# LiqunZhao/Neural-ordinary-differential-equations-based-Lyapunov-Barrier-Actor-Critic-NLBAC

Measured on AMD Instinct MI355X. Metric: ODE-integrate+update samples/sec, Unicycle batch 4096, higher is better.
Workload: dtype f32; 1 GPU; Unicycle B=4096 dopri5 (BASELINE.json configs[1] at B=4096 dopri5); NODE fit on 32768 rows every 10 updates; replay of 65536 synthetic transitions resident in HBM; solver=dopri5, adjoint=False, batch_per_gpu=4096, global_batch=4096, node_fit_rows_per_gpu=32768, parallelism=dp1, hipgraph=False

## Files before the change

### neural-ordinary-differential-equations-based-lyapunov-barrier-actor-critic-nlbac_amd/csrc/mlp_kernels.hip

```cpp
#include "common.h"
#include "mlp_device.h"
#include "rr_device.h"
#include "dy_heads.h"
#include "mlp_launch.h"


__global__ __launch_bounds__(256) void mlp_pack_kernel(const MlpLaunch L) {
    const nlbac_mlp& net = L.net[blockIdx.y];
    const int nwide = net.n_layers - 1;
    const int hid = net.hid;
    const long gid = (long)blockIdx.x * 256 + threadIdx.x;
    const long stride = (long)gridDim.x * 256;
    for (int l = 0; l < nwide; ++l) {
        const int K = (l == 0) ? net.in_dim : hid;
        const float* W = net.params + net.w_off[l];
        if (net.pf_off[l] >= 0) {
            const int KC = pad8(K) >> 3, NT = pad32(hid) >> 5;
            float* P = net.packed + net.pf_off[l];
            const long total = (long)NT * KC * 256;
            for (long i = gid; i < total; i += stride) {
                const int j = i & 3, lane = (i >> 2) & 63;
                const long tc = i >> 8;
                const int kc = tc % KC, tile = tc / KC;
                const int n = 32 * tile + (lane & 31), k = 8 * kc + 4 * (lane >> 5) + j;
// ... 396 lines not shown
    for (int r = 0; r < 16; ++r) acc[r] = 0.f;

#define DW_LOAD(r0_, A0, A1, B0, B1)                                                        \
    {                                                                                       \
        const int ra_ = min((r0_) + lr, re - 1), rb_ = min((r0_) + lr + 16, re - 1);        \
        A0 = *reinterpret_cast<const float4*>(pa + (long)ra_ * hid);                        \
        A1 = *reinterpret_cast<const float4*>(pa + (long)rb_ * hid);                        \
        B0 = *reinterpret_cast<const float4*>(pb + (long)ra_ * hid);                        \
        B1 = *reinterpret_cast<const float4*>(pb + (long)rb_ * hid);                        \
    }
#define DW_STAGE(r0_, A0, A1, B0, B1, buf_)                                                 \
    {                                                                                       \
        const bool lo_ = (r0_) + lr < re, hi_ = (r0_) + lr + 16 < re;                       \
        *reinterpret_cast<float4*>(&sA[buf_][lr][lc]) = sel4(a_ok && lo_, A0);              \
        *reinterpret_cast<float4*>(&sA[buf_][lr + 16][lc]) = sel4(a_ok && hi_, A1);         \
        *reinterpret_cast<float4*>(&sB[buf_][lr][lc]) = sel4(b_ok && lo_, B0);              \
        *reinterpret_cast<float4*>(&sB[buf_][lr + 16][lc]) = sel4(b_ok && hi_, B1);         \
    }
#define DW_MFMA(buf_)                                                                       \
    {                                                                                       \
        float av[DW_CHUNK / 2], bv[DW_CHUNK / 2];                                           \
        _Pragma("unroll") for (int bb = 0; bb < DW_CHUNK / 2; ++bb) {                       \
            av[bb] = sA[buf_][2 * bb + half][wn * 32 + (lane & 31)];                        \
            bv[bb] = sB[buf_][2 * bb + half][wk * 32 + (lane & 31)];                        \
        }                                                                                   \
        __builtin_amdgcn_sched_barrier(0);                                                  \
        _Pragma("unroll") for (int bb = 0; bb < DW_CHUNK / 2; ++bb)                         \
            acc = __builtin_amdgcn_mfma_f32_32x32x2f32(av[bb], bv[bb], acc, 0, 0, 0);       \
    }
    if (rb < re) {
        float4 x_a0, x_a1, x_b0, x_b1, y_a0, y_a1, y_b0, y_b1;
        DW_LOAD(rb, x_a0, x_a1, x_b0, x_b1)
        DW_STAGE(rb, x_a0, x_a1, x_b0, x_b1, 0)
        DW_LOAD(rb + DW_CHUNK, x_a0, x_a1, x_b0, x_b1)
        __syncthreads();
        for (int r0 = rb; r0 < re; r0 += 2 * DW_CHUNK) {
            if (r0 + 2 * DW_CHUNK < re) DW_LOAD(r0 + 2 * DW_CHUNK, y_a0, y_a1, y_b0, y_b1)
            __builtin_amdgcn_sched_barrier(0);
            DW_MFMA(0)
            __builtin_amdgcn_sched_barrier(0);
            if (r0 + DW_CHUNK < re) DW_STAGE(r0 + DW_CHUNK, x_a0, x_a1, x_b0, x_b1, 1)
            __syncthreads();
            if (r0 + DW_CHUNK >= re) break;
            if (r0 + 3 * DW_CHUNK < re) DW_LOAD(r0 + 3 * DW_CHUNK, x_a0, x_a1, x_b0, x_b1)
            __builtin_amdgcn_sched_barrier(0);
            DW_MFMA(1)
            __builtin_amdgcn_sched_barrier(0);
            if (r0 + 2 * DW_CHUNK < re) DW_STAGE(r0 + 2 * DW_CHUNK, y_a0, y_a1, y_b0, y_b1, 0)
            __syncthreads();
        }
    }
    float* g = io.grad + (long)slab * L.slab_stride + net.w_off[j];
    const int k = k0 + wk * 32 + (lane & 31);
#pragma unroll
    for (int r = 0; r < 16; ++r) {
        const int n = n0 + wn * 32 + acc_row(r, half);
        if (n < hid && k < hid) g[(long)n * hid + k] = acc[r];
    }
}

#define DWT_PF 8
__global__ __launch_bounds__(256, 3) void mlp_bwd_wide64_kernel(const MlpLaunch L, const SkinnyLaunch S,
                                                                const float* __restrict__ ws, int red_blocks,
                                                                int red_per_net, int n_nets, int tiles_per_group) {
    extern __shared__ __attribute__((aligned(16))) float dwt_smem[];
    if ((int)blockIdx.x < red_blocks) {
        const int inet = blockIdx.x / red_per_net;
        if (inet < n_nets)
            skinny_reduce_block(L, S, ws, blockIdx.x - inet * red_per_net, inet, reinterpret_cast<float (*)[64]>(dwt_smem));
        return;
    }
    const int id = (int)blockIdx.x - red_blocks, xcd = id & 7, jj = id >> 3;
    const int t = jj % tiles_per_group, grp = 8 * (jj / tiles_per_group) + xcd;
    if (grp >= L.n_slabs * n_nets) return;
    const int znet = grp / L.n_slabs, slab = grp - znet * L.n_slabs;
    const nlbac_mlp& net = L.net[znet];
    const nlbac_mlp_io& io = L.io[znet];
    const int B = L.B, hid = net.hid, nwide = net.n_layers - 1;
    const int T = (hid + 63) >> 6, per_layer = T * T;
    if (t >= (nwide - 1) * per_layer) return;
    const int j = 1 + t / per_layer, tt = t % per_layer;
    const int n0 = (tt / T) * 64, k0 = (tt % T) * 64;
    const int rb = slab * L.rows_per_slab, re = min(B, rb + L.rows_per_slab);
    const int tid = threadIdx.x, lane = tid & 63, wave = tid >> 6, q = lane >> 4, i = lane & 15;
    const long ls = io.acts_ls ? io.acts_ls : (long)B * hid;
    const __amdgpu_buffer_rsrc_t rsA = rr_rsrc(io.dz + (long)j * ls, max(re, 0) * hid);
    const __amdgpu_buffer_rsrc_t rsB = rr_rsrc(io.acts + (long)(j - 1) * ls, max(re, 0) * hid);
    const int oob = (int)0x80000000;
    const int voA = (n0 + 4 * i + 3 < hid) ? (q * hid + n0 + 4 * i) * 4 : oob;
    const int voB = (k0 + 4 * i + 3 < hid) ? (q * hid + k0 + 4 * i) * 4 : oob;
    const int kstep_bytes = 16 * hid;
    const int g_first = (rb >> 2) + wave, n_mine = (rb < re) ? (((re - rb + 3) >> 2) - wave + 3) / 4 : 0;
    f32x4 acc[4][4];
#pragma unroll
    for (int ta = 0; ta < 4; ++ta)
#pragma unroll
        for (int tb = 0; tb < 4; ++tb) acc[ta][tb] = f32x4{0.f, 0.f, 0.f, 0.f};
    f32x4 va[DWT_PF], vb[DWT_PF];
    const int rounds = (n_mine + DWT_PF - 1) / DWT_PF;
    if (rounds > 0) {
#pragma unroll
        for (int u = 0; u < DWT_PF; ++u) {
            const int so = (g_first + 4 * u) * kstep_bytes;
            va[u] = rr_ldw(rsA, voA, so);
            vb[u] = rr_ldw(rsB, voB, so);
        }
        int g = g_first + 4 * DWT_PF;
        for (int r = 0; r < rounds; ++r) {
#pragma unroll
            for (int u = 0; u < DWT_PF; ++u) {
                const f32x4 a = va[u], b = vb[u];
#pragma unroll
                for (int ta = 0; ta < 4; ++ta)
#pragma unroll
                    for (int tb = 0; tb < 4; ++tb)
                        acc[ta][tb] = __builtin_amdgcn_mfma_f32_16x16x4f32(a[ta], b[tb], acc[ta][tb], 0, 0, 0);
                const int so = g * kstep_bytes;
                va[u] = rr_ldw(rsA, voA, so);
                vb[u] = rr_ldw(rsB, voB, so);
                __builtin_amdgcn_sched_barrier(0);
                g += 4;
            }
        }
    }
    float* const red0 = dwt_smem, * const red1 = dwt_smem + 64 * 64;
    auto put = [&](float* red) __attribute__((always_inline)) {
#pragma unroll
        for (int ta = 0; ta < 4; ++ta)
#pragma unroll
            for (int tb = 0; tb < 4; ++tb)
                *reinterpret_cast<f32x4*>(red + ((ta * 4 + tb) * 64 + lane) * 4) = acc[ta][tb];
    };
    auto add = [&](const float* red) __attribute__((always_inline)) {
#pragma unroll
        for (int ta = 0; ta < 4; ++ta)
#pragma unroll
            for (int tb = 0; tb < 4; ++tb) acc[ta][tb] += *reinterpret_cast<const f32x4*>(red + ((ta * 4 + tb) * 64 + lane) * 4);
    };
    if (wave == 1) put(red0);
    if (wave == 3) put(red1);
    lds_barrier();
    if (wave == 0) add(red0);
    if (wave == 2) add(red1);
    lds_barrier();
    if (wave == 2) put(red0);
    lds_barrier();
    if (wave != 0) return;
    add(red0);
    float* gW = io.grad + (long)slab * L.slab_stride + net.w_off[j];
    if (k0 + 4 * i + 3 < hid) {
#pragma unroll
        for (int ta = 0; ta < 4; ++ta)
#pragma unroll
            for (int r = 0; r < 4; ++r) {
                const int n = n0 + 4 * (4 * q + r) + ta;
                if (n < hid)
                    *reinterpret_cast<f32x4*>(gW + (long)n * hid + k0 + 4 * i) = f32x4{acc[ta][0][r], acc[ta][1][r], acc[ta][2][r], acc[ta][3][r]};
            }
    }
}

#define DW128_LD 132
__global__ __launch_bounds__(256) void mlp_bwd_wide128_kernel(const MlpLaunch L) {
    extern __shared__ __attribute__((aligned(16))) float dw_smem[];
    float (*sA)[DW_CHUNK][DW128_LD] = reinterpret_cast<float (*)[DW_CHUNK][DW128_LD]>(dw_smem);
    float (*sB)[DW_CHUNK][DW128_LD] = reinterpret_cast<float (*)[DW_CHUNK][DW128_LD]>(dw_smem + 2 * DW_CHUNK * DW128_LD);
    const nlbac_mlp& net = L.net[blockIdx.z];
// ... 570 lines not shown
```

### neural-ordinary-differential-equations-based-lyapunov-barrier-actor-critic-nlbac_amd/csrc/node_adjoint_kernels.hip

```cpp
#include "node_adj_shared.h"

template <int MODE, int KEEP>
__global__ __launch_bounds__(512) void node_adj_kernel(const NodeAdjLaunch L) {
    extern __shared__ __attribute__((aligned(16))) float smem[];
    constexpr int BITS = KEEP ? 0 : 1;
    const int tid = threadIdx.x, t = tid & 255;
    const int grp = __builtin_amdgcn_readfirstlane(tid >> 8);
    const int lane = t & 63, wave = t >> 6;
    __shared__ unsigned s_gcnt[2];
    __shared__ int s_any;
    if (tid < 2) s_gcnt[tid] = 0u;
    if (tid == 2) s_any = 0;
    GroupBar gbar{&s_gcnt[grp], 0u, 4u};
    const int n = L.n, ns = L.n_s, nu = L.n_u, W = L.W, LD = L.ld, gout = ns * nu;
    const int row0 = blockIdx.x * NLBAC_MLP_TILE;
    const nlbac_mlp& net = L.net[grp];
    const int hid = net.hid, NT = pad32(hid) >> 5, hidp32 = NT * 32;
    const int nwide = net.n_layers - 1;
    const int inp = pad8(ns);
    const int n_rows = min(NLBAC_MLP_TILE, n - row0);
    const bool active = wave < NT, two = (MODE == 2) || (MODE == 0 && (wave + 4) < NT);

    float* buf = smem + grp * 2 * NLBAC_MLP_TILE * LD;
    float* sKZ = smem + 4 * NLBAC_MLP_TILE * LD;
// ... 332 lines not shown
                const float tol = atol + rtol * fmaxf(fabsf(z), fabsf(Z1[row * W + c]));
                const float q = a[row * W + c] / tol;
                v[part] += q * q;
            } else {
                const float sc = atol + fabsf(z) * rtol;
                if (mode == 0) {
                    const float q0 = z / sc, q1 = a[row * W + c] / sc;
                    v[part] += q0 * q0; v[part + 1] += q1 * q1;
                } else {
                    const float q = (a[row * W + c] - b[row * W + c]) / sc;
                    v[part] += q * q;
                }
            }
        }
        if (mode == 0)
            for (int c = 0; c < nu; ++c) {
                const float y = u[row * nu + c];
                const float q = y / (atol + fabsf(y) * rtol);
                v[0] += q * q;
            }
    }
    block_sum_256<4>(v, red);
    float* q = partials + ((long)p * gridDim.x + blockIdx.x) * 4;
    if (!publish) {
        if (threadIdx.x == 0)
            for (int k = 0; k < 4; ++k) q[k] = v[k];
        return;
    }
    if (threadIdx.x < 64) {
        float old = 0.f;
        if (threadIdx.x < 4) {
            const float mine = threadIdx.x == 0 ? v[0] : (threadIdx.x == 1 ? v[1] : (threadIdx.x == 2 ? v[2] : v[3]));
            old = __hip_atomic_exchange(q + threadIdx.x, mine, __ATOMIC_RELAXED, __HIP_MEMORY_SCOPE_AGENT);
        }
        asm volatile("" ::"v"(old) : "memory");
    }
}

__device__ __forceinline__ double max_keep_nan(double a, double b) { return (a != a || b != b) ? a + b : fmax(a, b); }
__device__ __forceinline__ float max_keep_nan(float a, float b) { return (a != a || b != b) ? a + b : fmaxf(a, b); }

__device__ __forceinline__ void adj_control_one(const double (&s)[4], int p, int mode, int ns, int nu, int rpp,
                                                double t_end, const float* pnorm, double* ctl) {
    const double cnt = (double)rpp * (double)(ns + nu);
    double n0 = max_keep_nan(sqrt(s[0] / cnt), sqrt(s[2] / cnt)), n1 = max_keep_nan(sqrt(s[1] / cnt), sqrt(s[3] / cnt));
    if (pnorm) { n0 = max_keep_nan(n0, (double)pnorm[0]); n1 = max_keep_nan(n1, (double)pnorm[1]); }
    dopri_control_vals(n0, n1, p, mode, t_end, ctl);
}

__global__ __launch_bounds__(256) void adj_norm_control_kernel(const float* a, const float* b, const float* Z0,
                                                               const float* Z1, const float* u, int mode, float rtol,
                                                               float atol, int ns, int nu, int rpp, double t_end,
                                                               const float* pnorm, float* partials, unsigned* tickets,
                                                               double* ctl, double* ctl_host, double host_seq) {
    const int p = blockIdx.y, nblk = (int)gridDim.x;
    if (mode == 2 && ctl[(long)p * NLBAC_DOPRI_CTL + C_DONE] > 0.0) return;
    adj_norm_block(a, b, Z0, Z1, u, mode, rtol, atol, ns, nu, rpp, partials, tickets != nullptr);
    if (!tickets) return;
    __shared__ unsigned s_last;
    __shared__ double s_red[4][256];
    if (threadIdx.x == 0) {
        elect_release_();
        const unsigned ticket = __hip_atomic_fetch_add(tickets + p, 1u, __ATOMIC_RELAXED, __HIP_MEMORY_SCOPE_AGENT);
        s_last = (ticket == gridDim.x - 1) ? 1u : 0u;
        if (s_last) __hip_atomic_store(tickets + p, 0u, __ATOMIC_RELAXED, __HIP_MEMORY_SCOPE_AGENT);
    }
    __syncthreads();
    if (!s_last) return;
    elect_acquire_();
    double v[4] = {0.0, 0.0, 0.0, 0.0};
    for (int bb = threadIdx.x; bb < nblk; bb += 256) {
        const float* q = partials + ((long)p * nblk + bb) * 4;
        for (int k = 0; k < 4; ++k) v[k] += (double)__hip_atomic_load(q + k, __ATOMIC_RELAXED, __HIP_MEMORY_SCOPE_AGENT);
    }
    for (int k = 0; k < 4; ++k) s_red[k][threadIdx.x] = v[k];
    __syncthreads();
    for (int w = 128; w >= 1; w >>= 1) {
        if ((int)threadIdx.x < w)
            for (int k = 0; k < 4; ++k) s_red[k][threadIdx.x] += s_red[k][threadIdx.x + w];
        __syncthreads();
    }
    if (threadIdx.x == 0) {
        const double s[4] = {s_red[0][0], s_red[1][0], s_red[2][0], s_red[3][0]};
        adj_control_one(s, p, mode, ns, nu, rpp, t_end, pnorm, ctl);
        if (ctl_host) ctl_host_post(ctl_host + (long)p * NLBAC_DOPRI_CTL, ctl + (long)p * NLBAC_DOPRI_CTL, host_seq);
    }
}

__global__ void adj_control_kernel(const float* partials, int nblk, int mode, int ns, int nu, int rpp, double t_end,
                                   const float* pnorm, double* ctl) {
    if (threadIdx.x != 0) return;
    const int p = blockIdx.x;
    if (mode == 2 && ctl[(long)p * NLBAC_DOPRI_CTL + C_DONE] > 0.0) return;
    double s[4] = {0.0, 0.0, 0.0, 0.0};
    for (int bb = 0; bb < nblk; ++bb)
        for (int k = 0; k < 4; ++k) s[k] += (double)partials[((long)p * nblk + bb) * 4 + k];
    adj_control_one(s, p, mode, ns, nu, rpp, t_end, pnorm, ctl);
}

extern "C" int nlbac_adj_norm_control(const float* a, const float* b, const float* Z0, const float* Z1, const float* u,
                                      int mode, float rtol, float atol, int n_s, int n_u, int rows_per_problem, int P,
                                      double t_end, const float* pnorm, float* partials, unsigned* tickets, double* ctl,
                                      double* ctl_host, double host_seq, nlbac_stream_t s) {
    NLBAC_REQUIRE(a && Z0 && partials && ctl && mode >= 0 && mode <= 2, "nlbac_adj_norm_control: bad arguments");
    NLBAC_REQUIRE((mode != 0 || u) && (mode != 1 || b) && (mode != 2 || Z1), "nlbac_adj_norm_control: missing operand");
    NLBAC_REQUIRE(P >= 1 && P <= 8, "nlbac_adj_norm_control: P %d out of range", P);
    hipLaunchKernelGGL(adj_norm_control_kernel, dim3(nlbac_ceil_div(rows_per_problem, 256), P), dim3(256), 0,
                       (hipStream_t)s, a, b, Z0, Z1, u, mode, rtol, atol, n_s, n_u, rows_per_problem, t_end, pnorm,
                       partials, tickets, ctl, tickets ? ctl_host : nullptr, host_seq);
    NLBAC_CHECK_LAUNCH("nlbac_adj_norm_control");
    return 0;
}

extern "C" int nlbac_adj_control(const float* partials, int n_blk_per_problem, int mode, int n_s, int n_u,
                                 int rows_per_problem, int P, double t_end, const float* pnorm, double* ctl,
                                 nlbac_stream_t s) {
    NLBAC_REQUIRE(partials && ctl && mode >= 0 && mode <= 2, "nlbac_adj_control: bad arguments");
    hipLaunchKernelGGL(adj_control_kernel, dim3(P), dim3(64), 0, (hipStream_t)s, partials, n_blk_per_problem, mode, n_s,
                       n_u, rows_per_problem, t_end, pnorm, ctl);
    NLBAC_CHECK_LAUNCH("nlbac_adj_control");
    return 0;
}

__global__ __launch_bounds__(256) void adj_commit_kernel(const double* ctl, int rpp, long n, int w, float* dst0,
                                                         const float* src0, float* dst1, const float* src1) {
    const long i = (long)blockIdx.x * 256 + threadIdx.x;
    if (i >= n) return;
    const double* c = ctl + (i / rpp) * NLBAC_DOPRI_CTL;
    if (!(c[C_ACCEPT] > 0.0) || c[C_DONE] > 0.0) return;
    for (int k = 0; k < w; ++k) {
        dst0[i * w + k] = src0[i * w + k];
        if (dst1) dst1[i * w + k] = src1[i * w + k];
    }
}

extern "C" int nlbac_adj_commit(const double* ctl, int rows_per_problem, long n_rows, int w, float* dst0,
                                const float* src0, float* dst1, const float* src1, nlbac_stream_t s) {
    NLBAC_REQUIRE(ctl && dst0 && src0 && n_rows >= 1 && w >= 1 && rows_per_problem >= 1 && (!dst1 || src1),
                  "nlbac_adj_commit: bad arguments");
    hipLaunchKernelGGL(adj_commit_kernel, dim3(nlbac_ceil_div(n_rows, 256)), dim3(256), 0, (hipStream_t)s, ctl,
                       rows_per_problem, n_rows, w, dst0, src0, dst1, src1);
    NLBAC_CHECK_LAUNCH("nlbac_adj_commit");
    return 0;
}

struct AdjParamArg { float c_sol[ADJ_MAX_STAGES]; float c_err[ADJ_MAX_STAGES]; int S; float h_host; };

__global__ __launch_bounds__(256) void adj_param_norm_kernel(int mode, const float* th0, const float* K, long stride,
                                                             const AdjParamArg A, const double* h_dev,
                                                             const int* seg_off, const int* seg_len, int n_seg,
                                                             float rtol, float atol, const double* ctl, float* th1,
                                                             float* pseg, unsigned* ticket, float* pnorm) {
    if (mode == 2 && ctl && ctl[C_DONE] > 0.0) return;
    __shared__ float red[8];
    __shared__ unsigned s_last;
    const int seg = blockIdx.x, off = seg_off[seg], len = seg_len[seg];
    const float h = h_dev ? (float)h_dev[0] : A.h_host;
    float v[2] = {0.f, 0.f};
    for (int i = threadIdx.x; i < len; i += 256) {
        const long e = off + i;
        const float z0 = th0[e];
        if (mode == 0) {
            const float sc = atol + fabsf(z0) * rtol;
            const float q0 = z0 / sc, q1 = K[e] / sc;
            v[0] += q0 * q0; v[1] += q1 * q1;
        } else if (mode == 1) {
            const float sc = atol + fabsf(z0) * rtol;
            const float q = (K[stride + e] - K[e]) / sc;
// ... 53 lines not shown
```

### neural-ordinary-differential-equations-based-lyapunov-barrier-actor-critic-nlbac_amd/csrc/ode_control.h

```cpp
#pragma once
#include "common.h"

enum { C_H = 0, C_T = 1, C_RATIO = 2, C_ACCEPT = 3, C_DONE = 4, C_X = 5, C_H0 = 6, C_D0 = 7, C_D1 = 8, C_D2 = 9,
       C_NSTEPS = 10, C_HUSED = 11,
       C_NACC = 12,
       C_OVF = 13 };

enum { C_SEQ = 15 };

__device__ __forceinline__ void ctl_host_post(double* dst, const double* src, double seq) {
    if (seq <= 0.0) {
        for (int k = 0; k < NLBAC_DOPRI_CTL; ++k) dst[k] = src[k];
        return;
    }
    double v[NLBAC_DOPRI_CTL];
    for (int k = 0; k < NLBAC_DOPRI_CTL; ++k) v[k] = src[k];
    __hip_atomic_store(dst + C_SEQ, -seq, __ATOMIC_RELAXED, __HIP_MEMORY_SCOPE_SYSTEM);
    asm volatile("s_waitcnt vmcnt(0)" ::: "memory");
    for (int k = 0; k < NLBAC_DOPRI_CTL; ++k)
        if (k != C_SEQ) __hip_atomic_store(dst + k, v[k], __ATOMIC_RELAXED, __HIP_MEMORY_SCOPE_SYSTEM);
    asm volatile("s_waitcnt vmcnt(0)" ::: "memory");
    __hip_atomic_store(dst + C_SEQ, seq, __ATOMIC_RELAXED, __HIP_MEMORY_SCOPE_SYSTEM);
}

__device__ __forceinline__ void dopri_control_vals(double n0, double n1, int p, int mode, double t_end, double* ctl,
                                                   int n_slots = 1 << 30) {
    double* c = ctl + (long)p * NLBAC_DOPRI_CTL;
    if (mode == 0) {
        const double d0 = n0, d1 = n1;
        c[C_D0] = d0; c[C_D1] = d1;
        c[C_H0] = (d0 < 1e-5 || d1 < 1e-5) ? 1e-6 : 0.01 * d0 / d1;
        c[C_T] = 0.0; c[C_NSTEPS] = 0.0; c[C_DONE] = 0.0; c[C_NACC] = 0.0; c[C_OVF] = 0.0;
    } else if (mode == 1) {
        const double h0 = c[C_H0], d1 = c[C_D1];
        const double d2 = n0 / h0;
        c[C_D2] = d2;
        double h1;
        if (d1 <= 1e-15 && d2 <= 1e-15) h1 = fmax(1e-6, h0 * 1e-3);
        else h1 = pow(0.01 / fmax(d1, d2), 1.0 / 5.0);
        c[C_H] = fmin(100.0 * h0, h1);
    } else {
        const double ratio = n0;
        const double h = c[C_H], t = c[C_T];
        const bool accept = ratio <= 1.0;
        double fac;
        if (ratio == 0.0) fac = 10.0;
        else {
            const double dfac = (ratio < 1.0) ? 1.0 : 0.2;
            fac = fmin(10.0, fmax(0.9 / pow(ratio, 0.2), dfac));
        }
        c[C_RATIO] = ratio; c[C_ACCEPT] = accept ? 1.0 : 0.0; c[C_HUSED] = h;
        c[C_NSTEPS] += 1.0;
        if (accept && t + h >= t_end) {
            c[C_DONE] = 1.0;
            c[C_X] = (t_end - t) / h;
        } else {
            if (accept) {
                c[C_T] = t + h;
                if ((int)c[C_NACC] + 1 >= n_slots) { c[C_OVF] = 1.0; c[C_DONE] = 1.0; }
                else c[C_NACC] += 1.0;
            }
            c[C_H] = h * fac;
        }
    }
}

#define DPM0 (6025192743.0 / 30085553152.0 / 2.0)
#define DPM2 (51252292925.0 / 65400821598.0 / 2.0)
#define DPM3 (-2691868925.0 / 45128329728.0 / 2.0)
#define DPM4 (187940372067.0 / 1594534317056.0 / 2.0)
#define DPM5 (-1776094331.0 / 19743644256.0 / 2.0)
#define DPM6 (11237099.0 / 235043384.0 / 2.0)

__device__ __forceinline__ float dopri_interp_value(float a0, float a1, const float (&k)[7], float h, float x) {
#pragma clang fp contract(off)
    const float cm[7] = {(float)DPM0, 0.f, (float)DPM2, (float)DPM3, (float)DPM4, (float)DPM5, (float)DPM6};
    float ym = a0;
#pragma unroll
    for (int j = 0; j < 7; ++j)
        if (cm[j] != 0.f) ym = ym + k[j] * (cm[j] * h);
    const float f0 = k[0], f1 = k[6];
    const float a = 2.f * h * (f1 - f0) - 8.f * (a1 + a0) + 16.f * ym;
    const float b = h * (5.f * f0 - 3.f * f1) + 18.f * a0 + 14.f * a1 - 32.f * ym;
    const float c = h * (f1 - 4.f * f0) - 11.f * a0 - 5.f * a1 + 16.f * ym;
    const float d = h * f0;
    return a0 + x * (d + x * (c + x * (b + x * a)));
}

__device__ __forceinline__ void dopri_interp_grad(float g, float h, float x, float& dy0, float& dy1, float (&dk)[7]) {
#pragma clang fp contract(off)
    const float cm[7] = {(float)DPM0, 0.f, (float)DPM2, (float)DPM3, (float)DPM4, (float)DPM5, (float)DPM6};
    const float x2 = x * x, x3 = x2 * x, x4 = x2 * x2;
    const float A = x4 * g, Bc = x3 * g, C = x2 * g, D = x * g;
    const float ym = 16.f * A - 32.f * Bc + 16.f * C;
    dy0 = g - 8.f * A + 18.f * Bc - 11.f * C + ym;
    dy1 = -8.f * A + 14.f * Bc - 5.f * C;
    const float f0b = h * (-2.f * A + 5.f * Bc - 4.f * C + D);
    const float f1b = h * (2.f * A - 3.f * Bc + C);
#pragma unroll
    for (int j = 0; j < 7; ++j) {
        float v = (cm[j] * h) * ym;
        if (j == 0) v += f0b;
        if (j == 6) v += f1b;
        dk[j] = v;
    }
// ... 2 lines not shown
```

### neural-ordinary-differential-equations-based-lyapunov-barrier-actor-critic-nlbac_amd/csrc/ode_kernels.hip

```cpp
#include "common.h"
#include "ode_control.h"

#define MAX_NS 8
#define MAX_NUA 4
#define MAX_STAGES 8
#define MAX_PROBLEMS 8

struct RkCoef { float c[MAX_STAGES]; float h[MAX_PROBLEMS]; };

__device__ __forceinline__ float step_of(const RkCoef& rc, const double* h_dev, int h_stride, int p) {
    return h_dev ? (float)h_dev[(long)p * h_stride] : rc.h[p];
}

__global__ __launch_bounds__(256) void affine_fwd_kernel(const float* f, const float* g, const float* u, int n_s,
                                                         int n_u, int n, float* k) {
    const int i = blockIdx.x * 256 + threadIdx.x;
    if (i >= n) return;
    for (int r = 0; r < n_s; ++r) {
        float a = f[(long)i * n_s + r];
        for (int c = 0; c < n_u; ++c) a += g[(long)i * n_s * n_u + r * n_u + c] * u[(long)i * n_u + c];
        k[(long)i * n_s + r] = a;
    }
}

// ... 65 lines not shown
        for (int r = 0; r < n_s; ++r) {
            const float y = y0[row * n_s + r];
            if (mode == 2) {
                const float tol = atol + rtol * fmaxf(fabsf(y), fabsf(y1[row * n_s + r]));
                const float q = a[row * n_s + r] / tol;
                v[0] += q * q;
            } else {
                const float sc = atol + fabsf(y) * rtol;
                if (mode == 0) {
                    const float q0 = y / sc, q1 = a[row * n_s + r] / sc;
                    v[0] += q0 * q0; v[1] += q1 * q1;
                } else {
                    const float q = (a[row * n_s + r] - b[row * n_s + r]) / sc;
                    v[0] += q * q;
                }
            }
        }
        if (mode == 0)
            for (int c = 0; c < n_u; ++c) {
                const float y = u[row * n_u + c];
                const float q = y / (atol + fabsf(y) * rtol);
                v[0] += q * q;
            }
    }
    block_sum_256<2>(v, red);
    float* q = partials + ((long)p * gridDim.x + blockIdx.x) * 2;
    if (!publish) {
        if (threadIdx.x == 0) { q[0] = v[0]; q[1] = v[1]; }
        return;
    }
    if (threadIdx.x < 64) {
        float old = 0.f;
        if (threadIdx.x < 2) old = __hip_atomic_exchange(q + threadIdx.x, threadIdx.x ? v[1] : v[0], __ATOMIC_RELAXED, __HIP_MEMORY_SCOPE_AGENT);
        asm volatile("" ::"v"(old) : "memory");
    }
}

__global__ __launch_bounds__(256) void dopri_norm_kernel(const float* a, const float* b, const float* y0,
                                                         const float* y1, const float* u, int mode, float rtol,
                                                         float atol, int n_s, int n_u, int rpp, float* partials,
                                                         const double* slot_ctl, long slot_floats) {
    if (slot_ctl && mode == 2 && slot_ctl[(long)blockIdx.y * NLBAC_DOPRI_CTL + C_DONE] > 0.0) return;
    dopri_norm_block(a, b, y0, y1, u, mode, rtol, atol, n_s, n_u, rpp, partials, slot_ctl, slot_floats);
}

__device__ __forceinline__ void dopri_control_one(double s0, double s1, int p, int mode, int n_s, int n_u,
                                                  int rpp, double t_end, double* ctl) {
    const double cnt = (double)rpp * (double)(n_s + n_u);
    dopri_control_vals(sqrt(s0 / cnt), sqrt(s1 / cnt), p, mode, t_end, ctl);
}

__global__ void dopri_control_kernel(const float* partials, int nblk, int mode, int n_s, int n_u, int rpp,
                                     double t_end, double* ctl, int n_slots, double* hslots, double* alog,
                                     int alog_cap) {
    if (threadIdx.x != 0) return;
    const int p = blockIdx.x;
    double* c = ctl + (long)p * NLBAC_DOPRI_CTL;
    if (n_slots > 0 && mode == 2 && c[C_DONE] > 0.0) return;
    double s0 = 0.0, s1 = 0.0;
    for (int b = 0; b < nblk; ++b) {
        s0 += (double)partials[((long)p * nblk + b) * 2 + 0];
        s1 += (double)partials[((long)p * nblk + b) * 2 + 1];
    }
    const int slot_before = (int)c[C_NACC];
    const double h_try = c[C_H];
    const double cnt = (double)rpp * (double)(n_s + n_u);
    dopri_control_vals(sqrt(s0 / cnt), sqrt(s1 / cnt), p, mode, t_end, ctl, n_slots > 0 ? n_slots : (1 << 30));
    if (hslots && mode == 2 && c[C_ACCEPT] > 0.0) hslots[(long)p * n_slots + slot_before] = h_try;
    if (alog && mode == 2) {
        const int k = (int)c[C_NSTEPS] - 1;
        if (k >= 0 && k < alog_cap) {
            double* a = alog + ((long)p * alog_cap + k) * 3;
            a[0] = h_try; a[1] = c[C_RATIO]; a[2] = c[C_ACCEPT];
        }
    }
}

__global__ __launch_bounds__(64) void dopri_control_tiles_kernel(const float* partials, int nblk, int n_s, int n_u, int rpp,
                                                                 double t_end, double* ctl, int n_slots, double* hslots,
                                                                 double* alog, int alog_cap, double* ctl_host,
                                                                 double host_seq) {
    const int p = blockIdx.x, tid = threadIdx.x;
    double* c = ctl + (long)p * NLBAC_DOPRI_CTL;
    if (c[C_DONE] > 0.0) return;
    double d0 = 0.0, d1 = 0.0;
    for (int b = tid; b < nblk; b += 64) {
        const float* q = partials + ((long)p * nblk + b) * 2;
        d0 += (double)q[0];
        d1 += (double)q[1];
    }
#pragma unroll
    for (int off = 32; off > 0; off >>= 1) { d0 += __shfl_down(d0, off, 64); d1 += __shfl_down(d1, off, 64); }
    if (tid != 0) return;
    const int slot_before = (int)c[C_NACC];
    const double h_try = c[C_H];
    const double cnt = (double)rpp * (double)(n_s + n_u);
    dopri_control_vals(sqrt(d0 / cnt), sqrt(d1 / cnt), p, 2, t_end, ctl, n_slots > 0 ? n_slots : (1 << 30));
    if (hslots && c[C_ACCEPT] > 0.0) hslots[(long)p * n_slots + slot_before] = h_try;
    if (alog) {
        const int k = (int)c[C_NSTEPS] - 1;
        if (k >= 0 && k < alog_cap) {
            double* al = alog + ((long)p * alog_cap + k) * 3;
            al[0] = h_try; al[1] = c[C_RATIO]; al[2] = c[C_ACCEPT];
        }
    }
    if (ctl_host) ctl_host_post(ctl_host + (long)p * NLBAC_DOPRI_CTL, c, host_seq);
}

__global__ __launch_bounds__(256) void dopri_norm_control_kernel(const float* a, const float* b, const float* y0,
                                                                 const float* y1, const float* u, int mode, float rtol,
                                                                 float atol, int n_s, int n_u, int rpp, double t_end,
                                                                 float* partials, unsigned* tickets, double* ctl,
                                                                 const double* slot_ctl, long slot_floats, int n_slots,
                                                                 double* hslots, double* alog, int alog_cap,
                                                                 double* ctl_host, double host_seq) {
    if (slot_ctl && mode == 2 && slot_ctl[(long)blockIdx.y * NLBAC_DOPRI_CTL + C_DONE] > 0.0) return;
    dopri_norm_block(a, b, y0, y1, u, mode, rtol, atol, n_s, n_u, rpp, partials, slot_ctl, slot_floats, true);
    __shared__ unsigned s_last;
    __shared__ double s_red[2][256];
    const int p = blockIdx.y, nblk = (int)gridDim.x;
    if (threadIdx.x == 0) {
        const unsigned ticket = __hip_atomic_fetch_add(tickets + p, 1u, __ATOMIC_RELAXED, __HIP_MEMORY_SCOPE_AGENT);
        s_last = (ticket == gridDim.x - 1) ? 1u : 0u;
        if (s_last) __hip_atomic_store(tickets + p, 0u, __ATOMIC_RELAXED, __HIP_MEMORY_SCOPE_AGENT);
    }
    __syncthreads();
    if (!s_last) return;
    double v0 = 0.0, v1 = 0.0;
    for (int b = threadIdx.x; b < nblk; b += 256) {
        const float* q = partials + ((long)p * nblk + b) * 2;
        v0 += (double)__hip_atomic_load(q + 0, __ATOMIC_RELAXED, __HIP_MEMORY_SCOPE_AGENT);
        v1 += (double)__hip_atomic_load(q + 1, __ATOMIC_RELAXED, __HIP_MEMORY_SCOPE_AGENT);
    }
    s_red[0][threadIdx.x] = v0;
    s_red[1][threadIdx.x] = v1;
    __syncthreads();
    for (int w = 128; w >= 1; w >>= 1) {
        if ((int)threadIdx.x < w) {
            s_red[0][threadIdx.x] += s_red[0][threadIdx.x + w];
            s_red[1][threadIdx.x] += s_red[1][threadIdx.x + w];
        }
        __syncthreads();
    }
    if (threadIdx.x == 0) {
        double* c = ctl + (long)p * NLBAC_DOPRI_CTL;
        const int slot_before = (int)c[C_NACC];
        const double h_try = c[C_H];
        const double cnt = (double)rpp * (double)(n_s + n_u);
        dopri_control_vals(sqrt(s_red[0][0] / cnt), sqrt(s_red[1][0] / cnt), p, mode, t_end, ctl,
                           n_slots > 0 ? n_slots : (1 << 30));
        if (hslots && mode == 2 && c[C_ACCEPT] > 0.0) hslots[(long)p * n_slots + slot_before] = h_try;
        if (alog && mode == 2) {
            const int k = (int)c[C_NSTEPS] - 1;
            if (k >= 0 && k < alog_cap) {
                double* al = alog + ((long)p * alog_cap + k) * 3;
                al[0] = h_try; al[1] = c[C_RATIO]; al[2] = c[C_ACCEPT];
            }
        }
        if (ctl_host) ctl_host_post(ctl_host + (long)p * NLBAC_DOPRI_CTL, c, host_seq);
    }
}

struct InterpArg { float h[MAX_PROBLEMS]; float x[MAX_PROBLEMS]; const double* ctl; long slot_floats; };

__device__ __forceinline__ int interp_slot(const InterpArg& ia, int p) {
    return (ia.ctl && ia.slot_floats) ? (int)ia.ctl[(long)p * NLBAC_DOPRI_CTL + C_NACC] : 0;
}

__device__ __forceinline__ void interp_hx(const InterpArg& ia, int p, float& h, float& x) {
    if (ia.ctl) {
        h = (float)ia.ctl[(long)p * NLBAC_DOPRI_CTL + C_HUSED];
        x = (float)ia.ctl[(long)p * NLBAC_DOPRI_CTL + C_X];
    } else {
        h = ia.h[p]; x = ia.x[p];
    }
}

struct OutMap { int kind; float l; float* p; const float* dp; const float* dp2; const float* x; };

__global__ __launch_bounds__(256) void dopri_interp_fwd_kernel(const float* y0, const float* y1, const float* K,
                                                               const InterpArg ia, int rpp, int n_s, int n,
                                                               float* out, const OutMap om) {
    const int i = blockIdx.x * 256 + threadIdx.x;
    if (i >= n) return;
    float h, x;
    interp_hx(ia, i / rpp, h, x);
    {
        const int slot = interp_slot(ia, i / rpp);
        y1 += (long)slot * ia.slot_floats;
        K += (long)slot * ia.slot_floats;
        if (slot > 0) y0 = y1 - ia.slot_floats;
    }
    for (int r = 0; r < n_s; ++r) {
        float k[7];
#pragma unroll
        for (int j = 0; j < 7; ++j) k[j] = K[((long)j * n + i) * n_s + r];
        out[(long)i * n_s + r] = dopri_interp_value(y0[(long)i * n_s + r], y1[(long)i * n_s + r], k, h, x);
    }
    if (om.kind == 1) {
        const float th = out[(long)i * n_s + 2];
        om.p[i * 2 + 0] = out[(long)i * n_s + 0] + om.l * cosf(th);
        om.p[i * 2 + 1] = out[(long)i * n_s + 1] + om.l * sinf(th);
    }
}

__global__ __launch_bounds__(256) void dopri_interp_bwd_kernel(const float* dout, const InterpArg ia, int rpp,
                                                               int n_s, int n, float* dy0, float* dy1, float* dK,
                                                               const OutMap om) {
    const int i = blockIdx.x * 256 + threadIdx.x;
    if (i >= n) return;
    float h, x;
    interp_hx(ia, i / rpp, h, x);
    {
        const long off = (long)interp_slot(ia, i / rpp) * ia.slot_floats;
        dy0 += off; dy1 += off; dK += off;
    }
    float gm[3] = {0.f, 0.f, 0.f};
    if (om.kind == 1) {
        float d0 = om.dp[i * 2 + 0], d1 = om.dp[i * 2 + 1];
        if (om.dp2) { d0 += om.dp2[i * 2 + 0]; d1 += om.dp2[i * 2 + 1]; }
        const float th = om.x[(long)i * n_s + 2];
        gm[0] = d0; gm[1] = d1; gm[2] = om.l * (-sinf(th) * d0 + cosf(th) * d1);
    }
    for (int r = 0; r < n_s; ++r) {
        const float g = (om.kind == 1) ? gm[r] : dout[(long)i * n_s + r];
        float d0v, d1v, dk[7];
        dopri_interp_grad(g, h, x, d0v, d1v, dk);
        dy0[(long)i * n_s + r] = d0v;
        dy1[(long)i * n_s + r] = d1v;
#pragma unroll
        for (int j = 0; j < 7; ++j) dK[((long)j * n + i) * n_s + r] = dk[j];
    }
}

#define GRID1(n) dim3(nlbac_ceil_div((n), 256)), dim3(256), 0, (hipStream_t)s

static int fill_rc(RkCoef& rc, const float* coef, int n_k, const float* h_host, int P, const char* who) {
    NLBAC_REQUIRE(n_k >= 0 && n_k <= MAX_STAGES, "%s: n_k %d out of range", who, n_k);
    NLBAC_REQUIRE(P >= 1 && P <= MAX_PROBLEMS, "%s: P %d out of range", who, P);
    memset(&rc, 0, sizeof(rc));
    for (int j = 0; j < n_k; ++j) rc.c[j] = coef[j];
    for (int p = 0; p < P; ++p) rc.h[p] = h_host ? h_host[p] : 1.f;
// ... 318 lines not shown
```

### neural-ordinary-differential-equations-based-lyapunov-barrier-actor-critic-nlbac_amd/csrc/optim_kernels.hip

```cpp
#include <cstdint>
#include "common.h"
#include "philox.h"

thread_local char nlbac_err_buf[512] = "";

extern "C" int nlbac_abi_version(void) { return NLBAC_ABI_VERSION; }
extern "C" const char* nlbac_last_error(void) { return nlbac_err_buf; }

struct AdamState {
    int step;
    float step_size;
    float bc2_sqrt;
    unsigned ticket;
};

__global__ void adam_prepare_kernel(AdamState* st, double lr) {
    if (threadIdx.x == 0 && blockIdx.x == 0) {
        const int t = st->step + 1;
        st->step = t;
        const double bc1 = 1.0 - pow(0.9, (double)t);
        const double bc2 = 1.0 - pow(0.999, (double)t);
        st->step_size = (float)(lr / bc1);
        st->bc2_sqrt = (float)sqrt(bc2);
    }
// ... 135 lines not shown
            scatter2(scat, 4 * i + 0, pp.x); scatter2(scat, 4 * i + 1, pp.y);
            scatter2(scat, 4 * i + 2, pp.z); scatter2(scat, 4 * i + 3, pp.w);
        }
        if (target) {
            float4 t = reinterpret_cast<float4*>(target)[i];
            t.x = t.x * (1.0f - tau) + pp.x * tau; t.y = t.y * (1.0f - tau) + pp.y * tau;
            t.z = t.z * (1.0f - tau) + pp.z * tau; t.w = t.w * (1.0f - tau) + pp.w * tau;
            reinterpret_cast<float4*>(target)[i] = t;
            if (scat_t) {
                scatter2(scat_t, 4 * i + 0, t.x); scatter2(scat_t, 4 * i + 1, t.y);
                scatter2(scat_t, 4 * i + 2, t.z); scatter2(scat_t, 4 * i + 3, t.w);
            }
        }
    }
    for (long i = (n4 << 2) + (long)blockIdx.x * blockDim.x + threadIdx.x; i < n; i += stride) {
        float g = grad[i];
        for (int s = 1; s < n_slabs; ++s) g += grad[s * slab_stride + i];
        float pp = p[i], mm = m[i], vv = v[i];
        adam_one(pp, mm, vv, g, step_size, bc2_sqrt);
        p[i] = pp; m[i] = mm; v[i] = vv;
        alpha_refresh(AR, i, pp);
        if (scat) scatter2(scat, i, pp);
        if (target) {
            const float t = target[i] * (1.0f - tau) + pp * tau;
            target[i] = t;
            if (scat_t) scatter2(scat_t, i, t);
        }
    }
    __syncthreads();
    __shared__ int s_is_last;
    if (threadIdx.x == 0) {
        s_is_last = 0;
        const unsigned ticket = __hip_atomic_fetch_add(&st->ticket, 1u, __ATOMIC_RELAXED, __HIP_MEMORY_SCOPE_AGENT);
        if (ticket == gridDim.x - 1) {
            __hip_atomic_store(&st->ticket, 0u, __ATOMIC_RELAXED, __HIP_MEMORY_SCOPE_AGENT);
            st->step_size = step_size;
            st->bc2_sqrt = bc2_sqrt;
            __hip_atomic_store(&st->step, s_step, __ATOMIC_RELAXED, __HIP_MEMORY_SCOPE_AGENT);
            s_is_last = 1;
        }
    }
    if (!AR.mirror_dst) return;
    __syncthreads();
    if (s_is_last)
        for (int i = threadIdx.x; i < AR.n_mirror; i += blockDim.x) {
            const bool refreshed = (AR.off[0] >= 0 && AR.dst[0] == AR.mirror_src + i) ||
                                   (AR.off[1] >= 0 && AR.dst[1] == AR.mirror_src + i);
            if (!refreshed) AR.mirror_dst[i] = AR.mirror_src[i];
        }
}

__global__ __launch_bounds__(256) void reduce_slabs_kernel(float* __restrict__ out, const float* __restrict__ grad,
                                                           int n_slabs, long slab_stride, long n) {
    const long stride = (long)gridDim.x * blockDim.x;
    for (long i = (long)blockIdx.x * blockDim.x + threadIdx.x; i < n; i += stride) {
        float g = grad[i];
        for (int s = 1; s < n_slabs; ++s) g += grad[s * slab_stride + i];
        out[i] = g;
    }
}

__global__ __launch_bounds__(256) void soft_update_kernel(float* __restrict__ target, const float* __restrict__ src,
                                                          long n, float tau) {
    const long stride = (long)gridDim.x * blockDim.x;
    for (long i = (long)blockIdx.x * blockDim.x + threadIdx.x; i < n; i += stride)
        target[i] = target[i] * (1.0f - tau) + src[i] * tau;
}

__global__ __launch_bounds__(256) void axpby_kernel(float a, const float* x, float b, const float* y, long n, float* out) {
    const long stride = (long)gridDim.x * blockDim.x;
    for (long i = (long)blockIdx.x * blockDim.x + threadIdx.x; i < n; i += stride)
        out[i] = a * x[i] + (y ? b * y[i] : 0.f);
}

__global__ __launch_bounds__(256) void fill_kernel(float* p, float v, long n) {
    const long stride = (long)gridDim.x * blockDim.x;
    for (long i = (long)blockIdx.x * blockDim.x + threadIdx.x; i < n; i += stride) p[i] = v;
}

__global__ void sum_partials_kernel(const float* partials, int n_blk, int n_cols, float mul, float* out) {
    const int c = blockIdx.x * blockDim.x + threadIdx.x;
    if (c >= n_cols) return;
    float s = 0.f;
    for (int b = 0; b < n_blk; ++b) s += partials[(long)b * n_cols + c];
    out[c] = s * mul;
}

static inline int stream_grid(long n, int per_thread = 1) {
    long b = (n / per_thread + 255) / 256;
    if (b < 1) b = 1;
    if (b > 2048) b = 2048;
    return (int)b;
}

extern "C" int nlbac_adam_prepare(void* state, double lr, nlbac_stream_t s) {
    NLBAC_REQUIRE(state, "nlbac_adam_prepare: null state");
    hipLaunchKernelGGL(adam_prepare_kernel, dim3(1), dim3(64), 0, (hipStream_t)s, (AdamState*)state, lr);
    NLBAC_CHECK_LAUNCH("nlbac_adam_prepare");
    return 0;
}

extern "C" int nlbac_adam_step(float* p, float* m, float* v, const float* grad, int n_slabs, long slab_stride,
                               long n, const void* state, float* target, float tau, nlbac_stream_t s) {
    NLBAC_REQUIRE(p && m && v && grad && state, "nlbac_adam_step: null pointer");
    NLBAC_REQUIRE(n_slabs >= 1 && n >= 1, "nlbac_adam_step: bad sizes");
    NLBAC_REQUIRE(((uintptr_t)p | (uintptr_t)m | (uintptr_t)v | (uintptr_t)grad | (uintptr_t)target) % 16 == 0 &&
                      slab_stride % 4 == 0,
                  "nlbac_adam_step: buffers must be 16-byte aligned");
    hipLaunchKernelGGL(adam_step_kernel, dim3(stream_grid(n, 4)), dim3(256), 0, (hipStream_t)s, p, m, v, grad,
                       n_slabs, slab_stride, n, (const AdamState*)state, (tau >= 0.f) ? target : nullptr, tau);
    NLBAC_CHECK_LAUNCH("nlbac_adam_step");
    return 0;
}

extern "C" int nlbac_adam_fused(float* p, float* m, float* v, const float* grad, int n_slabs, long slab_stride, long n,
                                void* state, double lr, float* target, float tau, const void* scatter,
                                const void* scatter_target, int scatter_slots, int n_alpha, const long* alpha_off,
                                float* const* alpha_dst, const float* mirror_src, float* mirror_dst, int n_mirror,
                                nlbac_stream_t s) {
    NLBAC_REQUIRE(p && m && v && grad && state, "nlbac_adam_fused: null pointer");
    NLBAC_REQUIRE(scatter_slots == 2 || scatter_slots == 4 || (!scatter && !scatter_target),
                  "nlbac_adam_fused: scatter tables hold 2 or 4 slots per parameter");
    NLBAC_REQUIRE(n_alpha >= 0 && n_alpha <= 2 && (n_alpha == 0 || (alpha_off && alpha_dst)), "nlbac_adam_fused: bad alpha refresh");
    AlphaRefresh AR;
    AR.off[0] = AR.off[1] = -1; AR.dst[0] = AR.dst[1] = nullptr;
    NLBAC_REQUIRE((mirror_dst == nullptr) || (mirror_src && n_mirror > 0 && n_mirror <= 1024), "nlbac_adam_fused: bad mirror");
    AR.mirror_src = mirror_src; AR.mirror_dst = mirror_dst; AR.n_mirror = mirror_dst ? n_mirror : 0;
    for (int k = 0; k < n_alpha; ++k) {
        NLBAC_REQUIRE(alpha_off[k] >= 0 && alpha_off[k] < n && alpha_dst[k], "nlbac_adam_fused: alpha entry out of range");
        AR.off[k] = alpha_off[k]; AR.dst[k] = alpha_dst[k];
    }
    NLBAC_REQUIRE(n_slabs >= 1 && n >= 1 && lr > 0.0, "nlbac_adam_fused: bad sizes");
    NLBAC_REQUIRE(((uintptr_t)p | (uintptr_t)m | (uintptr_t)v | (uintptr_t)grad | (uintptr_t)target) % 16 == 0 &&
                      slab_stride % 4 == 0 && ((uintptr_t)scatter | (uintptr_t)scatter_target) % 16 == 0,
                  "nlbac_adam_fused: buffers must be 16-byte aligned");
    NLBAC_REQUIRE(!scatter_target || (target && tau >= 0.f), "nlbac_adam_fused: scatter_target without a target");
    hipLaunchKernelGGL((scatter_slots == 4 ? adam_fused_kernel<4> : adam_fused_kernel<2>), dim3(stream_grid(n, 4)), dim3(256),
                       0, (hipStream_t)s, p, m, v, grad, n_slabs, slab_stride, n, (AdamState*)state, lr,
                       (tau >= 0.f) ? target : nullptr, tau, (const unsigned long long*)scatter,
                       (const unsigned long long*)scatter_target, AR);
    NLBAC_CHECK_LAUNCH("nlbac_adam_fused");
    return 0;
}

extern "C" int nlbac_reduce_slabs(float* out, const float* grad, int n_slabs, long slab_stride, long n, nlbac_stream_t s) {
    NLBAC_REQUIRE(out && grad && n_slabs >= 1, "nlbac_reduce_slabs: bad arguments");
    hipLaunchKernelGGL(reduce_slabs_kernel, dim3(stream_grid(n)), dim3(256), 0, (hipStream_t)s, out, grad, n_slabs, slab_stride, n);
    NLBAC_CHECK_LAUNCH("nlbac_reduce_slabs");
    return 0;
}

extern "C" int nlbac_soft_update(float* target, const float* src, long n, float tau, nlbac_stream_t s) {
    NLBAC_REQUIRE(target && src, "nlbac_soft_update: null pointer");
    hipLaunchKernelGGL(soft_update_kernel, dim3(stream_grid(n)), dim3(256), 0, (hipStream_t)s, target, src, n, tau);
    NLBAC_CHECK_LAUNCH("nlbac_soft_update");
    return 0;
}

extern "C" int nlbac_axpby(float a, const float* x, float b, const float* y, long n, float* out, nlbac_stream_t s) {
    NLBAC_REQUIRE(x && out, "nlbac_axpby: null pointer");
    hipLaunchKernelGGL(axpby_kernel, dim3(stream_grid(n)), dim3(256), 0, (hipStream_t)s, a, x, b, y, n, out);
    NLBAC_CHECK_LAUNCH("nlbac_axpby");
    return 0;
}

extern "C" int nlbac_fill(float* p, float v, long n, nlbac_stream_t s) {
    NLBAC_REQUIRE(p, "nlbac_fill: null pointer");
// ... 190 lines not shown
```

Baseline: 3.701 million samples/s.

## Cache control state in registers and batch partial-sum loads in control kernels

The DOPRI step-control kernels now copy the per-problem control block into a local register array, run the step-size logic on it, and write it back once, so the host post no longer rereads global memory. The partial-sum reduction in the dopri control kernel issues several loads ahead per thread and broadcasts the control fields from one wave load via readlane. The optimizer's column reduction is unrolled by 16 for memory-level parallelism, and the dW kernel marks the wave index as wave-uniform. These target latency-bound serial loads in small control and reduction kernels, at the cost of more registers and clamped redundant loads.

```diff
diff --git a/neural-ordinary-differential-equations-based-lyapunov-barrier-actor-critic-nlbac_amd/csrc/mlp_kernels.hip b/neural-ordinary-differential-equations-based-lyapunov-barrier-actor-critic-nlbac_amd/csrc/mlp_kernels.hip
--- a/neural-ordinary-differential-equations-based-lyapunov-barrier-actor-critic-nlbac_amd/csrc/mlp_kernels.hip
+++ b/neural-ordinary-differential-equations-based-lyapunov-barrier-actor-critic-nlbac_amd/csrc/mlp_kernels.hip
@@ -502,7 +502,7 @@
     const int j = 1 + t / per_layer, tt = t % per_layer;
     const int n0 = (tt / T) * 64, k0 = (tt % T) * 64;
     const int rb = slab * L.rows_per_slab, re = min(B, rb + L.rows_per_slab);
-    const int tid = threadIdx.x, lane = tid & 63, wave = tid >> 6, q = lane >> 4, i = lane & 15;
+    const int tid = threadIdx.x, lane = tid & 63, wave = __builtin_amdgcn_readfirstlane(tid >> 6), q = lane >> 4, i = lane & 15;
     const long ls = io.acts_ls ? io.acts_ls : (long)B * hid;
     const __amdgpu_buffer_rsrc_t rsA = rr_rsrc(io.dz + (long)j * ls, max(re, 0) * hid);
     const __amdgpu_buffer_rsrc_t rsB = rr_rsrc(io.acts + (long)(j - 1) * ls, max(re, 0) * hid);
diff --git a/neural-ordinary-differential-equations-based-lyapunov-barrier-actor-critic-nlbac_amd/csrc/node_adjoint_kernels.hip b/neural-ordinary-differential-equations-based-lyapunov-barrier-actor-critic-nlbac_amd/csrc/node_adjoint_kernels.hip
--- a/neural-ordinary-differential-equations-based-lyapunov-barrier-actor-critic-nlbac_amd/csrc/node_adjoint_kernels.hip
+++ b/neural-ordinary-differential-equations-based-lyapunov-barrier-actor-critic-nlbac_amd/csrc/node_adjoint_kernels.hip
@@ -438,8 +438,11 @@
     }
     if (threadIdx.x == 0) {
         const double s[4] = {s_red[0][0], s_red[1][0], s_red[2][0], s_red[3][0]};
-        adj_control_one(s, p, mode, ns, nu, rpp, t_end, pnorm, ctl);
-        if (ctl_host) ctl_host_post(ctl_host + (long)p * NLBAC_DOPRI_CTL, ctl + (long)p * NLBAC_DOPRI_CTL, host_seq);
+        double loc[NLBAC_DOPRI_CTL];
+        ctl_load(loc, ctl + (long)p * NLBAC_DOPRI_CTL);
+        adj_control_one(s, 0, mode, ns, nu, rpp, t_end, pnorm, loc);
+        ctl_store(ctl + (long)p * NLBAC_DOPRI_CTL, loc);
+        if (ctl_host) ctl_host_post(ctl_host + (long)p * NLBAC_DOPRI_CTL, loc, host_seq);
     }
 }
 
diff --git a/neural-ordinary-differential-equations-based-lyapunov-barrier-actor-critic-nlbac_amd/csrc/ode_control.h b/neural-ordinary-differential-equations-based-lyapunov-barrier-actor-critic-nlbac_amd/csrc/ode_control.h
--- a/neural-ordinary-differential-equations-based-lyapunov-barrier-actor-critic-nlbac_amd/csrc/ode_control.h
+++ b/neural-ordinary-differential-equations-based-lyapunov-barrier-actor-critic-nlbac_amd/csrc/ode_control.h
@@ -8,19 +8,28 @@
 
 enum { C_SEQ = 15 };
 
-__device__ __forceinline__ void ctl_host_post(double* dst, const double* src, double seq) {
+__device__ __forceinline__ void ctl_host_post(double* dst, const double (&v)[NLBAC_DOPRI_CTL], double seq) {
     if (seq <= 0.0) {
-        for (int k = 0; k < NLBAC_DOPRI_CTL; ++k) dst[k] = src[k];
+#pragma unroll
+        for (int k = 0; k < NLBAC_DOPRI_CTL; ++k) dst[k] = v[k];
         return;
     }
-    double v[NLBAC_DOPRI_CTL];
-    for (int k = 0; k < NLBAC_DOPRI_CTL; ++k) v[k] = src[k];
     __hip_atomic_store(dst + C_SEQ, -seq, __ATOMIC_RELAXED, __HIP_MEMORY_SCOPE_SYSTEM);
     asm volatile("s_waitcnt vmcnt(0)" ::: "memory");
+#pragma unroll
     for (int k = 0; k < NLBAC_DOPRI_CTL; ++k)
         if (k != C_SEQ) __hip_atomic_store(dst + k, v[k], __ATOMIC_RELAXED, __HIP_MEMORY_SCOPE_SYSTEM);
     asm volatile("s_waitcnt vmcnt(0)" ::: "memory");
     __hip_atomic_store(dst + C_SEQ, seq, __ATOMIC_RELAXED, __HIP_MEMORY_SCOPE_SYSTEM);
+}
+
+__device__ __forceinline__ void ctl_load(double (&v)[NLBAC_DOPRI_CTL], const double* c) {
+#pragma unroll
+    for (int k = 0; k < NLBAC_DOPRI_CTL; ++k) v[k] = c[k];
+}
+__device__ __forceinline__ void ctl_store(double* c, const double (&v)[NLBAC_DOPRI_CTL]) {
+#pragma unroll
+    for (int k = 0; k < NLBAC_DOPRI_CTL; ++k) c[k] = v[k];
 }
 
 __device__ __forceinline__ void dopri_control_vals(double n0, double n1, int p, int mode, double t_end, double* ctl,
diff --git a/neural-ordinary-differential-equations-based-lyapunov-barrier-actor-critic-nlbac_amd/csrc/ode_kernels.hip b/neural-ordinary-differential-equations-based-lyapunov-barrier-actor-critic-nlbac_amd/csrc/ode_kernels.hip
--- a/neural-ordinary-differential-equations-based-lyapunov-barrier-actor-critic-nlbac_amd/csrc/ode_kernels.hip
+++ b/neural-ordinary-differential-equations-based-lyapunov-barrier-actor-critic-nlbac_amd/csrc/ode_kernels.hip
@@ -171,29 +171,54 @@
                                                                  double host_seq) {
     const int p = blockIdx.x, tid = threadIdx.x;
     double* c = ctl + (long)p * NLBAC_DOPRI_CTL;
-    if (c[C_DONE] > 0.0) return;
+    const double field = c[tid & (NLBAC_DOPRI_CTL - 1)];
+    constexpr int U = 4;
+    float q0[U], q1[U];
+    auto request = [&](int b0) __attribute__((always_inline)) {
+#pragma unroll
+        for (int u = 0; u < U; ++u) {
+            const int b = b0 + 64 * u;
+            if (b < nblk) {
+                const float* q = partials + ((long)p * nblk + b) * 2;
+                q0[u] = q[0];
+                q1[u] = q[1];
+            }
+        }
+    };
+    request(tid);
+    double loc[NLBAC_DOPRI_CTL];
+#pragma unroll
+    for (int k = 0; k < NLBAC_DOPRI_CTL; ++k)
+        loc[k] = __hiloint2double(__builtin_amdgcn_readlane(__double2hiint(field), k),
+                                  __builtin_amdgcn_readlane(__double2loint(field), k));
+    if (loc[C_DONE] > 0.0) return;
     double d0 = 0.0, d1 = 0.0;
-    for (int b = tid; b < nblk; b += 64) {
-        const float* q = partials + ((long)p * nblk + b) * 2;
-        d0 += (double)q[0];
-        d1 += (double)q[1];
+    for (int b0 = tid; b0 < nblk; b0 += 64 * U) {
+        if (b0 != tid) request(b0);
+#pragma unroll
+        for (int u = 0; u < U; ++u)
+            if (b0 + 64 * u < nblk) {
+                d0 += (double)q0[u];
+                d1 += (double)q1[u];
+            }
     }
 #pragma unroll
     for (int off = 32; off > 0; off >>= 1) { d0 += __shfl_down(d0, off, 64); d1 += __shfl_down(d1, off, 64); }
     if (tid != 0) return;
-    const int slot_before = (int)c[C_NACC];
-    const double h_try = c[C_H];
+    const int slot_before = (int)loc[C_NACC];
+    const double h_try = loc[C_H];
     const double cnt = (double)rpp * (double)(n_s + n_u);
-    dopri_control_vals(sqrt(d0 / cnt), sqrt(d1 / cnt), p, 2, t_end, ctl, n_slots > 0 ? n_slots : (1 << 30));
-    if (hslots && c[C_ACCEPT] > 0.0) hslots[(long)p * n_slots + slot_before] = h_try;
+    dopri_control_vals(sqrt(d0 / cnt), sqrt(d1 / cnt), 0, 2, t_end, loc, n_slots > 0 ? n_slots : (1 << 30));
+    ctl_store(c, loc);
+    if (hslots && loc[C_ACCEPT] > 0.0) hslots[(long)p * n_slots + slot_before] = h_try;
     if (alog) {
-        const int k = (int)c[C_NSTEPS] - 1;
+        const int k = (int)loc[C_NSTEPS] - 1;
         if (k >= 0 && k < alog_cap) {
             double* al = alog + ((long)p * alog_cap + k) * 3;
-            al[0] = h_try; al[1] = c[C_RATIO]; al[2] = c[C_ACCEPT];
-        }
-    }
-    if (ctl_host) ctl_host_post(ctl_host + (long)p * NLBAC_DOPRI_CTL, c, host_seq);
+            al[0] = h_try; al[1] = loc[C_RATIO]; al[2] = loc[C_ACCEPT];
+        }
+    }
+    if (ctl_host) ctl_host_post(ctl_host + (long)p * NLBAC_DOPRI_CTL, loc, host_seq);
 }
 
 __global__ __launch_bounds__(256) void dopri_norm_control_kernel(const float* a, const float* b, const float* y0,
@@ -232,21 +257,23 @@
         __syncthreads();
     }
     if (threadIdx.x == 0) {
-        double* c = ctl + (long)p * NLBAC_DOPRI_CTL;
-        const int slot_before = (int)c[C_NACC];
-        const double h_try = c[C_H];
+        double loc[NLBAC_DOPRI_CTL];
+        ctl_load(loc, ctl + (long)p * NLBAC_DOPRI_CTL);
+        const int slot_before = (int)loc[C_NACC];
+        const double h_try = loc[C_H];
         const double cnt = (double)rpp * (double)(n_s + n_u);
-        dopri_control_vals(sqrt(s_red[0][0] / cnt), sqrt(s_red[1][0] / cnt), p, mode, t_end, ctl,
+        dopri_control_vals(sqrt(s_red[0][0] / cnt), sqrt(s_red[1][0] / cnt), 0, mode, t_end, loc,
                            n_slots > 0 ? n_slots : (1 << 30));
-        if (hslots && mode == 2 && c[C_ACCEPT] > 0.0) hslots[(long)p * n_slots + slot_before] = h_try;
+        ctl_store(ctl + (long)p * NLBAC_DOPRI_CTL, loc);
+        if (hslots && mode == 2 && loc[C_ACCEPT] > 0.0) hslots[(long)p * n_slots + slot_before] = h_try;
         if (alog && mode == 2) {
-            const int k = (int)c[C_NSTEPS] - 1;
+            const int k = (int)loc[C_NSTEPS] - 1;
             if (k >= 0 && k < alog_cap) {
                 double* al = alog + ((long)p * alog_cap + k) * 3;
-                al[0] = h_try; al[1] = c[C_RATIO]; al[2] = c[C_ACCEPT];
+                al[0] = h_try; al[1] = loc[C_RATIO]; al[2] = loc[C_ACCEPT];
             }
         }
-        if (ctl_host) ctl_host_post(ctl_host + (long)p * NLBAC_DOPRI_CTL, c, host_seq);
+        if (ctl_host) ctl_host_post(ctl_host + (long)p * NLBAC_DOPRI_CTL, loc, host_seq);
     }
 }
 
diff --git a/neural-ordinary-differential-equations-based-lyapunov-barrier-actor-critic-nlbac_amd/csrc/optim_kernels.hip b/neural-ordinary-differential-equations-based-lyapunov-barrier-actor-critic-nlbac_amd/csrc/optim_kernels.hip
--- a/neural-ordinary-differential-equations-based-lyapunov-barrier-actor-critic-nlbac_amd/csrc/optim_kernels.hip
+++ b/neural-ordinary-differential-equations-based-lyapunov-barrier-actor-critic-nlbac_amd/csrc/optim_kernels.hip
@@ -241,7 +241,14 @@
     const int c = blockIdx.x * blockDim.x + threadIdx.x;
     if (c >= n_cols) return;
     float s = 0.f;
-    for (int b = 0; b < n_blk; ++b) s += partials[(long)b * n_cols + c];
+    for (int b0 = 0; b0 < n_blk; b0 += 16) {
+        float x[16];
+#pragma unroll
+        for (int k = 0; k < 16; ++k) x[k] = partials[(long)min(b0 + k, n_blk - 1) * n_cols + c];
+#pragma unroll
+        for (int k = 0; k < 16; ++k)
+            if (b0 + k < n_blk) s += x[k];
+    }
     out[c] = s * mul;
 }
 
```

New measurement: 3.715 million samples/s, median of 4. Within noise of the previous version (+0.4%).
